# TheoCoombes/ClipCap

Hardware: AMD Instinct MI355X
Metric: train samples/sec (512-d prefix, 40-tok caption) (higher is better)
Workload: dtype bf16; 1 GPU; BASELINE configs[1]: TransformerMapper(8L,P=L=10,H=8)+frozen GPT-2-small; per_gpu_batch=256, global_batch=256, encoder_dim=512, train_language_model=False, parallelism=dp1

## Files before the change

clipcap_amd/csrc/kernels.hip:

```cpp
#include "kernels.h"
#include "gemm_api.h"

namespace CC_NS {

__global__ void k_f32_to_bf16(const float* __restrict__ src, op16_t* __restrict__ dst, size_t n8) {
    for (size_t i = (size_t)blockIdx.x * blockDim.x + threadIdx.x; i < n8; i += (size_t)gridDim.x * blockDim.x) {
        const float4 a = reinterpret_cast<const float4*>(src)[2 * i], b = reinterpret_cast<const float4*>(src)[2 * i + 1];
        float v[8] = {a.x, a.y, a.z, a.w, b.x, b.y, b.z, b.w};
        reinterpret_cast<uint4*>(dst)[i] = pack8(v);
    }
}
int f32_to_bf16(const float* src, op16_t* dst, size_t n, hipStream_t st) {
    if (n & 7) return CC_ERR_SHAPE;
    const size_t n8 = n >> 3;
    if (!n8) return CC_OK;
    const int grid = (int)std::min<size_t>((n8 + 255) / 256, 2048);
    hipLaunchKernelGGL(k_f32_to_bf16, dim3(grid), dim3(256), 0, st, src, dst, n8);
    return CC_OK;
}

__device__ __forceinline__ unsigned short wire_bf16(float f) {
    const unsigned u = __float_as_uint(f);
    if ((u & 0x7fffffffu) > 0x7f800000u) return (unsigned short)((u >> 16) | 0x40u);
    return (unsigned short)((u + 0x7fffu + ((u >> 16) & 1u)) >> 16);
// ... 1046 lines not shown
                    const op16x8 a_h = frag_row_p(Dh + (blk * 32 + l31) * LDP + j * 32, t, half), a_l = frag_row_p(Dl + (blk * 32 + l31) * LDP + j * 32, t, half);
                    const op16x8 b_h = frag_tr_p<LD>(Kh + j * 32 * LD, nb, t, lane), b_l = frag_tr_p<LD>(Kl + j * 32 * LD, nb, t, lane);
                    CC_MFMA3(a_h, a_l, b_h, b_l, acc)
                }
        } else {
            const op16_t* Ah = kind == 1 ? Dh : Ph, *Al = kind == 1 ? Dl : Pl, *Bh = kind == 1 ? Qh : Oh, *Bl = kind == 1 ? Ql : Ol;
            for (int i = CAUSAL ? blk : 0; i < NBLK; i++)
#pragma unroll
                for (int t = 0; t < 2; t++) {
                    const op16x8 a_h = frag_tr_p<LDP>(Ah + i * 32 * LDP, blk, t, lane), a_l = frag_tr_p<LDP>(Al + i * 32 * LDP, blk, t, lane);
                    const op16x8 b_h = frag_tr_p<LD>(Bh + i * 32 * LD, nb, t, lane), b_l = frag_tr_p<LD>(Bl + i * 32 * LD, nb, t, lane);
                    CC_MFMA3(a_h, a_l, b_h, b_l, acc)
                }
        }
        const int d = nb * 32 + l31;
        if (img) {
            const int odd = lane & 1;
            op16_t* r3 = reinterpret_cast<op16_t*>(dqkv) + (size_t)b * S * 9 * D + kind * D + h * HD + (d & ~1);
#pragma unroll
            for (int rp = 0; rp < 8; rp++) {
                const float v0 = acc[2 * rp], v1 = acc[2 * rp + 1];
                const float got = __shfl_xor(odd ? v0 : v1, 1, 64);
                const float a0 = odd ? got : v0, a1 = odd ? v1 : got;
                const int row = blk * 32 + ((2 * rp) & 3) + 8 * ((2 * rp) >> 2) + 4 * half + odd;
                const unsigned hi = pack2op(a0, a1);
                float h0, h1;
                unpack2(hi, h0, h1);
                const unsigned lo = pack2op(a0 - h0, a1 - h1);
                if (row < S) {
                    op16_t* o3 = r3 + (size_t)row * 9 * D;
                    *reinterpret_cast<unsigned*>(o3) = hi;
                    *reinterpret_cast<unsigned*>(o3 + 3 * D) = hi;
                    *reinterpret_cast<unsigned*>(o3 + 6 * D) = lo;
                }
            }
        } else {
            float* o1 = dqkv + (size_t)b * S * rs + kind * D + h * HD + d;
#pragma unroll
            for (int r = 0; r < 16; r++) {
                const int row = blk * 32 + (r & 3) + 8 * (r >> 2) + 4 * half;
                if (row < S) o1[(size_t)row * rs] = acc[r];
            }
        }
    }
    __syncthreads();
    }
}
template <int HD, int NBLK>
static int attn_bwd_m3_launch(const float* qkv, const float* dout, const float* lse, int B, int S, int H, bool causal, float* dqkv, hipStream_t st,
                              Drop drop, int img) {
    typedef AttM3<HD, NBLK> G;
    const float scale = 1.0f / sqrtf((float)HD);
    static int ncu = 0;
    if (!ncu) {
        int dev = 0;
        hipDeviceProp_t pr;
        if (hipGetDevice(&dev) != hipSuccess || hipGetDeviceProperties(&pr, dev) != hipSuccess) return CC_ERR_STATE;
        ncu = pr.multiProcessorCount;
    }
    const int per_cu = (int)((size_t)160 * 1024 / G::lds);
    const dim3 grid(min(B * H, ncu * max(1, per_cu))), blk(64 * G::NW);
#define CC_M3_LAUNCH(C, DR)                                                                                                              \
    {                                                                                                                                    \
        if (G::lds > 64 * 1024) (void)hipFuncSetAttribute((const void*)k_attn_bwd_m3<HD, NBLK, C, DR>, hipFuncAttributeMaxDynamicSharedMemorySize, (int)G::lds); \
        hipLaunchKernelGGL((k_attn_bwd_m3<HD, NBLK, C, DR>), grid, blk, G::lds, st, qkv, dout, lse, B, S, H, scale, dqkv, drop, img);          \
    }
    if (drop.thresh) {
        if (!causal) return CC_ERR_SHAPE;
        CC_M3_LAUNCH(true, true)
    } else if (causal) CC_M3_LAUNCH(true, false)
    else CC_M3_LAUNCH(false, false)
#undef CC_M3_LAUNCH
    return hipGetLastError() == hipSuccess ? CC_OK : CC_ERR_LAUNCH;
}
static bool attn_x3mfma_on();
static bool attn_bwd_m3_ok(int S, int hd) { return attn_x3mfma_on() && (hd == 64 || hd == 96) && S > 0 && S <= 64; }
static bool attn_x3mfma_on() {
    static const bool on = !(cc_lab_env("CC_ATTN_X3MFMA") && atoi(cc_lab_env("CC_ATTN_X3MFMA")) == 0) && !cc_lab_env("CC_ATTN_F32MFMA");
    return on;
}
#endif

#if CC_OP != 2
template <int HD, bool CAUSAL, bool DROP = false>
__global__ __launch_bounds__(256, HD == 64 ? 3 : 2) void k_attn_fwd_mfma(const op16_t* __restrict__ qkv, int B, int S, int H, float scale,
                                                       op16_t* __restrict__ out, float* __restrict__ lse_out, Drop drop = Drop()) {
    constexpr int KK = HD / 16, NB = HD / 32, C8 = HD / 8;
    __shared__ __attribute__((aligned(16))) op16_t vsm[4][32 * AttLd<HD>::v];
    const int lane = threadIdx.x & 63, wave = threadIdx.x >> 6;
    const int nqb = (S + 31) >> 5;
    const int item = blockIdx.x * 4 + wave;
    if (item >= B * H * nqb) return;
    const int qb = item % nqb, h = (item / nqb) % H, b = item / (nqb * H);
    const int D = H * HD;
    const size_t rs = (size_t)3 * D;
    const op16_t* base = qkv + (size_t)b * S * rs + h * HD;
    const int half = lane >> 5, q = qb * 32 + (lane & 31);
    op16_t* vs = vsm[wave];

    op16x8 qf[KK];
#pragma unroll
    for (int kk = 0; kk < KK; kk++) {
        uint4 v = *reinterpret_cast<const uint4*>(base + (size_t)min(q, S - 1) * rs + kk * 16 + half * 8);
        if (q >= S) v = make_uint4(0, 0, 0, 0);
        qf[kk] = __builtin_bit_cast(op16x8, v);
    }
    f32x16 o[NB];
#pragma unroll
    for (int nb = 0; nb < NB; nb++)
#pragma unroll
        for (int r = 0; r < 16; r++) o[nb][r] = 0.f;
    float m = -INFINITY, l = 0.f;
    const int nkb = CAUSAL ? qb + 1 : nqb;
    uint4 kq[KK], vq[HD / 16];
    auto fetch = [&](int kb, uint4 (&kd)[KK], uint4 (&vd)[HD / 16]) {
        const int key = kb * 32 + (lane & 31);
#pragma unroll
        for (int kk = 0; kk < KK; kk++) {
            kd[kk] = *reinterpret_cast<const uint4*>(base + D + (size_t)min(key, S - 1) * rs + kk * 16 + half * 8);
            if (key >= S) kd[kk] = make_uint4(0, 0, 0, 0);
        }
#pragma unroll
        for (int c = 0; c < HD / 16; c++) {
            const int idx = lane + 64 * c;
            const int vk = idx / C8, vc = idx % C8;
            vd[c] = *reinterpret_cast<const uint4*>(base + 2 * D + (size_t)min(kb * 32 + vk, S - 1) * rs + vc * 8);
            if (kb * 32 + vk >= S) vd[c] = make_uint4(0, 0, 0, 0);
        }
    };
    fetch(0, kq, vq);
    for (int kb = 0; kb < nkb; kb++) {
        uint4 kn[KK], vn[HD / 16];
        fetch(kb + 1, kn, vn);
        f32x16 s;
#pragma unroll
        for (int r = 0; r < 16; r++) s[r] = 0.f;
#pragma unroll
        for (int kk = 0; kk < KK; kk++) s = CC_MFMA_32x32x16(__builtin_bit_cast(op16x8, kq[kk]), qf[kk], s);
#pragma unroll
        for (int c = 0; c < HD / 16; c++) {
            const int idx = lane + 64 * c;
            *reinterpret_cast<uint4*>(vs + (idx / C8) * AttLd<HD>::v + (idx % C8) * 8) = vq[c];
        }
        float mx = -INFINITY;
#pragma unroll
        for (int r = 0; r < 16; r++) {
            const int kr = kb * 32 + (r & 3) + 8 * (r >> 2) + 4 * half;
            const bool ok = kr < S && (!CAUSAL || kr <= q);
            s[r] = ok ? s[r] * scale : -INFINITY;
            mx = fmaxf(mx, s[r]);
        }
        mx = fmaxf(mx, __shfl_xor(mx, 32, 64));
        const float m_new = fmaxf(m, mx);
        const float alpha = (m == -INFINITY) ? 0.f : __expf(m - m_new);
        float p[16], ps = 0.f;
#pragma unroll
        for (int r = 0; r < 16; r++) {
            p[r] = (m_new == -INFINITY) ? 0.f : __expf(s[r] - m_new);
            ps += p[r];
        }
        ps += __shfl_xor(ps, 32, 64);
        l = l * alpha + ps;
        m = m_new;
#pragma unroll
        for (int nb = 0; nb < NB; nb++)
#pragma unroll
            for (int r = 0; r < 16; r++) o[nb][r] *= alpha;
        if (DROP) {
            const unsigned rowbase = ((unsigned)(b * H + h) * S + min(q, S - 1)) * S;
#pragma unroll
            for (int r = 0; r < 16; r++) p[r] *= drop_mul(drop, rowbase + min(kb * 32 + (r & 3) + 8 * (r >> 2) + 4 * half, S - 1));
        }
        op16x8 pf[2];
#pragma unroll
        for (int t = 0; t < 2; t++) {
            const uint4 v = make_uint4(pack2op(p[t * 8 + 0], p[t * 8 + 1]), pack2op(p[t * 8 + 2], p[t * 8 + 3]),
                                       pack2op(p[t * 8 + 4], p[t * 8 + 5]), pack2op(p[t * 8 + 6], p[t * 8 + 7]));
            pf[t] = __builtin_bit_cast(op16x8, v);
        }
#pragma unroll
        for (int t = 0; t < 2; t++)
#pragma unroll
            for (int nb = 0; nb < NB; nb++) o[nb] = CC_MFMA_32x32x16(frag_tr<HD>(vs, nb, t, lane), pf[t], o[nb]);
#pragma unroll
        for (int kk = 0; kk < KK; kk++) kq[kk] = kn[kk];
#pragma unroll
        for (int c = 0; c < HD / 16; c++) vq[c] = vn[c];
    }
    if (q < S) {
        const float inv = l > 0.f ? 1.f / l : 0.f;
        op16_t* orow = out + ((size_t)b * S + q) * D + h * HD;
#pragma unroll
        for (int nb = 0; nb < NB; nb++)
#pragma unroll
            for (int g = 0; g < 4; g++) {
                const int d0 = nb * 32 + 8 * g + 4 * half;
                *reinterpret_cast<uint2*>(orow + d0) = make_uint2(pack2op(o[nb][g * 4 + 0] * inv, o[nb][g * 4 + 1] * inv),
                                                                  pack2op(o[nb][g * 4 + 2] * inv, o[nb][g * 4 + 3] * inv));
            }
        if (half == 0 && lse_out) lse_out[((size_t)b * H + h) * S + q] = m + __logf(l);
    }
}

template <int HD>
static int attn_fwd_mfma_launch(const op16_t* qkv, int B, int S, int H, bool causal, op16_t* out, float* lse, hipStream_t st, Drop drop) {
    const int items = B * H * ((S + 31) / 32);
    const float scale = 1.0f / sqrtf((float)HD);
    if (drop.thresh) {
        if (!causal) return CC_ERR_SHAPE;
        hipLaunchKernelGGL((k_attn_fwd_mfma<HD, true, true>), dim3((items + 3) / 4), dim3(256), 0, st, qkv, B, S, H, scale, out, lse, drop);
    } else if (causal)
        hipLaunchKernelGGL((k_attn_fwd_mfma<HD, true>), dim3((items + 3) / 4), dim3(256), 0, st, qkv, B, S, H, scale, out, lse, drop);
    else
        hipLaunchKernelGGL((k_attn_fwd_mfma<HD, false>), dim3((items + 3) / 4), dim3(256), 0, st, qkv, B, S, H, scale, out, lse, drop);
    return hipGetLastError() == hipSuccess ? CC_OK : CC_ERR_LAUNCH;
}

__device__ __forceinline__ op16x8 pack_frag(const float* p) {
    return __builtin_bit_cast(op16x8, make_uint4(pack2op(p[0], p[1]), pack2op(p[2], p[3]), pack2op(p[4], p[5]), pack2op(p[6], p[7])));
}
__device__ __forceinline__ op16x8 load_frag(const op16_t* row_ptr, bool ok) {
    uint4 v = *reinterpret_cast<const uint4*>(row_ptr);
    if (!ok) v = make_uint4(0, 0, 0, 0);
    return __builtin_bit_cast(op16x8, v);
}

template <int HD, bool CAUSAL, bool DROP = false>
__global__ __launch_bounds__(256, HD == 64 ? 2 : 1) void k_attn_bwd_dkv(const op16_t* __restrict__ qkv, const op16_t* __restrict__ dout,
                                                      const float* __restrict__ lse, const float* __restrict__ delta, int B, int S, int H,
                                                      float scale, op16_t* __restrict__ dqkv, Drop drop = Drop()) {
    constexpr int KK = HD / 16, NB = HD / 32;
    __shared__ __attribute__((aligned(16))) op16_t qsm[4][32 * AttLd<HD>::v];
    __shared__ __attribute__((aligned(16))) op16_t dsm[4][32 * AttLd<HD>::v];
    __shared__ __attribute__((aligned(16))) float ldsm[4][64];
    const int lane = threadIdx.x & 63, wave = threadIdx.x >> 6;
    const int nblk = (S + 31) >> 5;
    const int item = blockIdx.x * 4 + wave;
    if (item >= B * H * nblk) return;
    const int j = item % nblk, h = (item / nblk) % H, b = item / (nblk * H);
    const int D = H * HD;
    const size_t rs = (size_t)3 * D;
    const op16_t* base = qkv + (size_t)b * S * rs + h * HD;
    const op16_t* dbase = dout + (size_t)b * S * D + h * HD;
    const float* lrow = lse + ((size_t)b * H + h) * S;
    const float* drow = delta + ((size_t)b * H + h) * S;
    const int half = lane >> 5, key = j * 32 + (lane & 31);
    op16x8 kf[KK], vf[KK];
#pragma unroll
    for (int kk = 0; kk < KK; kk++) {
        kf[kk] = load_frag(base + D + (size_t)min(key, S - 1) * rs + kk * 16 + half * 8, key < S);
        vf[kk] = load_frag(base + 2 * D + (size_t)min(key, S - 1) * rs + kk * 16 + half * 8, key < S);
    }
    f32x16 dk[NB], dv[NB];
#pragma unroll
    for (int nb = 0; nb < NB; nb++)
#pragma unroll
        for (int r = 0; r < 16; r++) { dk[nb][r] = 0.f; dv[nb][r] = 0.f; }
    const int i0 = CAUSAL ? j : 0;
    op16x8 qf[KK], df[KK];
    {
        const int qa = i0 * 32 + (lane & 31);
#pragma unroll
        for (int kk = 0; kk < KK; kk++) {
            qf[kk] = load_frag(base + (size_t)min(qa, S - 1) * rs + kk * 16 + half * 8, qa < S);
            df[kk] = load_frag(dbase + (size_t)min(qa, S - 1) * D + kk * 16 + half * 8, qa < S);
        }
    }
    for (int i = i0; i < nblk; i++) {
        op16x8 qn[KK], dn[KK];
        {
            const int qa = (i + 1) * 32 + (lane & 31);
#pragma unroll
            for (int kk = 0; kk < KK; kk++) {
                qn[kk] = load_frag(base + (size_t)min(qa, S - 1) * rs + kk * 16 + half * 8, qa < S);
                dn[kk] = load_frag(dbase + (size_t)min(qa, S - 1) * D + kk * 16 + half * 8, qa < S);
            }
        }
        f32x16 s, dp;
#pragma unroll
        for (int r = 0; r < 16; r++) { s[r] = 0.f; dp[r] = 0.f; }
#pragma unroll
        for (int kk = 0; kk < KK; kk++) {
            s = CC_MFMA_32x32x16(qf[kk], kf[kk], s);
            dp = CC_MFMA_32x32x16(df[kk], vf[kk], dp);
            *reinterpret_cast<op16x8*>(qsm[wave] + (lane & 31) * AttLd<HD>::v + kk * 16 + half * 8) = qf[kk];
            *reinterpret_cast<op16x8*>(dsm[wave] + (lane & 31) * AttLd<HD>::v + kk * 16 + half * 8) = df[kk];
        }
        {
            const int qq = min(i * 32 + (lane & 31), S - 1);
            ldsm[wave][lane] = half ? drow[qq] : lrow[qq];
        }
        float lq[16], dq_[16];
// ... 81 lines not shown
#pragma unroll
    for (int nb = 0; nb < NB; nb++)
#pragma unroll
        for (int r = 0; r < 16; r++) dq[nb][r] = 0.f;
    const int jend = CAUSAL ? i + 1 : nblk;
    op16x8 kf[KK], vf[KK];
    {
        const int key = lane & 31;
#pragma unroll
        for (int kk = 0; kk < KK; kk++) {
            kf[kk] = load_frag(base + D + (size_t)min(key, S - 1) * rs + kk * 16 + half * 8, key < S);
            vf[kk] = load_frag(base + 2 * D + (size_t)min(key, S - 1) * rs + kk * 16 + half * 8, key < S);
        }
    }
    for (int j = 0; j < jend; j++) {
        op16x8 kn[KK], vn[KK];
        {
            const int key = (j + 1) * 32 + (lane & 31);
#pragma unroll
            for (int kk = 0; kk < KK; kk++) {
                kn[kk] = load_frag(base + D + (size_t)min(key, S - 1) * rs + kk * 16 + half * 8, key < S);
                vn[kk] = load_frag(base + 2 * D + (size_t)min(key, S - 1) * rs + kk * 16 + half * 8, key < S);
            }
        }
        f32x16 st, dpt;
#pragma unroll
        for (int r = 0; r < 16; r++) { st[r] = 0.f; dpt[r] = 0.f; }
#pragma unroll
        for (int kk = 0; kk < KK; kk++) {
            st = CC_MFMA_32x32x16(kf[kk], qf[kk], st);
            dpt = CC_MFMA_32x32x16(vf[kk], dof[kk], dpt);
            *reinterpret_cast<op16x8*>(ksm[wave] + (lane & 31) * AttLd<HD>::v + kk * 16 + half * 8) = kf[kk];
        }
        float ds[16];
#pragma unroll
        for (int r = 0; r < 16; r++) {
            const int kr = j * 32 + (r & 3) + 8 * (r >> 2) + 4 * half;
            const bool ok = kr < S && q < S && (!CAUSAL || kr <= q);
            const float p = ok ? __expf(st[r] * scale - my_lse) : 0.f;
            const float mk = DROP ? drop_mul(drop, ((unsigned)(b * H + h) * S + min(q, S - 1)) * S + min(kr, S - 1)) : 1.0f;
            ds[r] = p * (mk * dpt[r] - my_delta) * scale;
        }
        const op16x8 dsf[2] = {pack_frag(ds), pack_frag(ds + 8)};
#pragma unroll
        for (int t = 0; t < 2; t++)
#pragma unroll
            for (int nb = 0; nb < NB; nb++)
                dq[nb] = CC_MFMA_32x32x16(frag_tr<HD>(ksm[wave], nb, t, lane), dsf[t], dq[nb]);
#pragma unroll
        for (int kk = 0; kk < KK; kk++) { kf[kk] = kn[kk]; vf[kk] = vn[kk]; }
    }
    if (q < S) {
        op16_t* orow = dqkv + ((size_t)b * S + q) * rs + h * HD;
#pragma unroll
        for (int nb = 0; nb < NB; nb++)
#pragma unroll
            for (int g = 0; g < 4; g++) {
                const int d0 = nb * 32 + 8 * g + 4 * half;
                *reinterpret_cast<uint2*>(orow + d0) =
                    make_uint2(pack2op(dq[nb][g * 4 + 0], dq[nb][g * 4 + 1]), pack2op(dq[nb][g * 4 + 2], dq[nb][g * 4 + 3]));
            }
    }
}

#ifndef CC_ATTN_FUSED_OCC
#define CC_ATTN_FUSED_OCC 2
#endif
template <int LD, int ROWS = 32>
__device__ __forceinline__ op16x8 frag_tr_ld(const op16_t* blk, int nb, int t, int lane) {
    typedef __attribute__((ext_vector_type(4))) short s16x4_t;
    typedef __attribute__((address_space(3))) s16x4_t* lp_t;
    const int half = lane >> 5, j = lane & 15, dsub = (lane >> 4) & 1;
    const int r0 = 16 * t + 4 * half + (j >> 2);
    const op16_t* col = blk + nb * 32 + 16 * dsub + 4 * (j & 3);
    const op16_t* p = col + (ROWS < 32 ? min(r0, ROWS - 1) : r0) * LD;
    const op16_t* ph = col + (ROWS < 32 ? min(r0 + 8, ROWS - 1) : r0 + 8) * LD;
    const s16x4_t lo = __builtin_amdgcn_ds_read_tr16_b64_v4i16((lp_t)p);
    const s16x4_t hi = __builtin_amdgcn_ds_read_tr16_b64_v4i16((lp_t)ph);
    typedef __attribute__((ext_vector_type(8))) short s16x8_t;
    const s16x8_t v = {lo[0], lo[1], lo[2], lo[3], hi[0], hi[1], hi[2], hi[3]};
    return __builtin_bit_cast(op16x8, v);
}

template <int HD>
__device__ __forceinline__ void attn_store_tile(op16_t* T, const f32x16 (&acc)[HD / 32], op16_t* gblock, size_t gstride, int rows_left, int lane) {
    constexpr int LD = AttLd<HD>::v, C8 = HD / 8;
    const int half = lane >> 5, l31 = lane & 31;
#pragma unroll
    for (int nb = 0; nb < HD / 32; nb++)
#pragma unroll
        for (int g = 0; g < 4; g++)
            *reinterpret_cast<uint2*>(T + l31 * LD + nb * 32 + 8 * g + 4 * half) =
                make_uint2(pack2op(acc[nb][g * 4 + 0], acc[nb][g * 4 + 1]), pack2op(acc[nb][g * 4 + 2], acc[nb][g * 4 + 3]));
#pragma unroll
    for (int it = 0; it < C8 / 2; it++) {
        const int idx = lane + 64 * it, row = idx / C8, chunk = idx % C8;
        const uint4 v = *reinterpret_cast<const uint4*>(T + row * LD + chunk * 8);
        if (row < rows_left) *reinterpret_cast<uint4*>(gblock + (size_t)row * gstride + chunk * 8) = v;
    }
}

template <int HD, bool CAUSAL, bool DROP, int NBLK, int OCC, int DR = 32>
__global__ __launch_bounds__(256, OCC) void k_attn_bwd_fused(const op16_t* __restrict__ qkv, const op16_t* __restrict__ dout, const op16_t* __restrict__ o,
                                                             const float* __restrict__ lse, int B, int S, int H, float scale,
                                                             op16_t* __restrict__ dqkv, Drop drop = Drop()) {
    constexpr int KK = HD / 16, NB = HD / 32, LD = AttLd<HD>::v;
    constexpr bool SPARE = LD >= HD + 32;
    constexpr int LT = SPARE ? LD : 32;
    __shared__ __attribute__((aligned(16))) op16_t ksm[4][32 * LD];
    __shared__ __attribute__((aligned(16))) op16_t qsm[4][32 * LD];
    __shared__ __attribute__((aligned(16))) op16_t dsm[4][32 * LD];
    static_assert(DR == 32 || (!SPARE && NBLK == 1), "the short dS^T tile is for the single-block form with its own tile");
    __shared__ __attribute__((aligned(16))) op16_t dtx[SPARE ? 1 : 4][SPARE ? 8 : DR * 32];
    __shared__ __attribute__((aligned(16))) float ldsm[4][NBLK][64];
    const int lane = threadIdx.x & 63, wave = threadIdx.x >> 6;
    const int item = blockIdx.x * 4 + wave;
    if (item >= B * H) return;
    const int h = item % H, b = item / H;
    const int D = H * HD;
    const size_t rs = (size_t)3 * D;
    const op16_t* base = qkv + (size_t)b * S * rs + h * HD;
    const op16_t* dbase = dout + (size_t)b * S * D + h * HD;
    const op16_t* obase = o + (size_t)b * S * D + h * HD;
    const float* lrow = lse + ((size_t)b * H + h) * S;
    const int half = lane >> 5, l31 = lane & 31;
    const int coff = half * 8;
    op16_t* dtm = SPARE ? ksm[wave] + HD : dtx[SPARE ? 0 : wave];

    op16x8 qf[KK], dof[KK], kf[KK], vf[KK];
    auto load_q = [&](int i) {
        const int q = i * 32 + l31, qc = min(q, S - 1);
#pragma unroll
        for (int kk = 0; kk < KK; kk++) {
            qf[kk] = load_frag(base + (size_t)qc * rs + kk * 16 + coff, q < S);
            dof[kk] = load_frag(dbase + (size_t)qc * D + kk * 16 + coff, q < S);
        }
    };
    auto load_k = [&](int j) {
        const int key = j * 32 + l31, kc = min(key, S - 1);
#pragma unroll
        for (int kk = 0; kk < KK; kk++) {
            kf[kk] = load_frag(base + D + (size_t)kc * rs + kk * 16 + coff, key < S);
            vf[kk] = load_frag(base + 2 * D + (size_t)kc * rs + kk * 16 + coff, key < S);
        }
    };
    load_k(0);
    load_q(0);
#pragma unroll
    for (int i = 0; i < NBLK; i++) {
        const int q = i * 32 + l31, qc = min(q, S - 1);
        float acc = 0.f;
#pragma unroll
        for (int kk = 0; kk < KK; kk++) {
            const op16x8 df = load_frag(dbase + (size_t)qc * D + kk * 16 + coff, q < S);
            const op16x8 of = load_frag(obase + (size_t)qc * D + kk * 16 + coff, q < S);
            float x[8], y[8];
            unpack8(__builtin_bit_cast(uint4, df), x);
            unpack8(__builtin_bit_cast(uint4, of), y);
#pragma unroll
            for (int e = 0; e < 8; e++) acc += x[e] * y[e];
        }
        acc += __shfl_xor(acc, 32, 64);
        ldsm[wave][i][lane] = half ? acc : lrow[qc];
    }
    f32x16 dq[NBLK][NB];

#pragma unroll
    for (int j = 0; j < NBLK; j++) {
        const int key = j * 32 + l31;
#pragma unroll
        for (int kk = 0; kk < KK; kk++) *reinterpret_cast<op16x8*>(ksm[wave] + l31 * LD + kk * 16 + coff) = kf[kk];
        f32x16 dk[NB], dv[NB];
#pragma unroll
        for (int nb = 0; nb < NB; nb++)
#pragma unroll
            for (int r = 0; r < 16; r++) { dk[nb][r] = 0.f; dv[nb][r] = 0.f; }
#pragma unroll
        for (int i = 0; i < NBLK; i++) {
            if (CAUSAL && i < j) continue;
            const int ifirst = CAUSAL ? j : 0;
            if (!(j > 0 && i == ifirst && i == NBLK - 1)) {
#pragma unroll
                for (int kk = 0; kk < KK; kk++) {
                    *reinterpret_cast<op16x8*>(qsm[wave] + l31 * LD + kk * 16 + coff) = qf[kk];
                    *reinterpret_cast<op16x8*>(dsm[wave] + l31 * LD + kk * 16 + coff) = dof[kk];
                }
            }
            f32x16 s, dp;
#pragma unroll
            for (int r = 0; r < 16; r++) { s[r] = 0.f; dp[r] = 0.f; }
#pragma unroll
            for (int kk = 0; kk < KK; kk++) {
                s = CC_MFMA_32x32x16(qf[kk], kf[kk], s);
                dp = CC_MFMA_32x32x16(dof[kk], vf[kk], dp);
            }
            if (i + 1 < NBLK) {
                load_q(i + 1);
            } else if (j + 1 < NBLK) {
                const int ni = CAUSAL ? j + 1 : 0;
                if (ni != i) load_q(ni);
                load_k(j + 1);
            }
            if (j == 0) {
#pragma unroll
                for (int nb = 0; nb < NB; nb++)
#pragma unroll
                    for (int r = 0; r < 16; r++) dq[i][nb][r] = 0.f;
            }
            float p[16], ds[16];
#pragma unroll
            for (int g4 = 0; g4 < 4; g4++) {
                const float4 lq = *reinterpret_cast<const float4*>(&ldsm[wave][i][4 * half + 8 * g4]);
                const float4 dl = *reinterpret_cast<const float4*>(&ldsm[wave][i][32 + 4 * half + 8 * g4]);
                const float lqa[4] = {lq.x, lq.y, lq.z, lq.w}, dla[4] = {dl.x, dl.y, dl.z, dl.w};
#pragma unroll
                for (int e = 0; e < 4; e++) {
                    const int r = g4 * 4 + e;
                    const int qr = i * 32 + e + 8 * g4 + 4 * half;
                    const bool ok = qr < S && key < S && (!CAUSAL || key <= qr);
                    p[r] = ok ? __expf(s[r] * scale - lqa[e]) : 0.f;
                    if (DROP) {
                        const float mk = drop_mul(drop, ((unsigned)(b * H + h) * S + min(qr, S - 1)) * S + min(key, S - 1));
                        ds[r] = p[r] * (mk * dp[r] - dla[e]) * scale;
                        p[r] *= mk;
                    } else {
                        ds[r] = p[r] * (dp[r] - dla[e]) * scale;
                    }
                }
            }
            const op16x8 pf[2] = {pack_frag(p), pack_frag(p + 8)};
            const op16x8 dsf[2] = {pack_frag(ds), pack_frag(ds + 8)};
            if (DR == 32 || l31 < DR) {
#pragma unroll
                for (int t = 0; t < 2; t++) {
                    const uint4 w = __builtin_bit_cast(uint4, dsf[t]);
                    *reinterpret_cast<uint2*>(dtm + l31 * LT + 16 * t + 4 * half) = make_uint2(w.x, w.y);
                    *reinterpret_cast<uint2*>(dtm + l31 * LT + 16 * t + 8 + 4 * half) = make_uint2(w.z, w.w);
                }
            }
#pragma unroll
            for (int t = 0; t < 2; t++)
#pragma unroll
                for (int nb = 0; nb < NB; nb++) {
                    dv[nb] = CC_MFMA_32x32x16(frag_tr<HD>(dsm[wave], nb, t, lane), pf[t], dv[nb]);
                    dk[nb] = CC_MFMA_32x32x16(frag_tr<HD>(qsm[wave], nb, t, lane), dsf[t], dk[nb]);
                }
#pragma unroll
            for (int t = 0; t < 2; t++) {
                const op16x8 dst = frag_tr_ld<LT, DR>(dtm, 0, t, lane);
#pragma unroll
                for (int nb = 0; nb < NB; nb++) dq[i][nb] = CC_MFMA_32x32x16(frag_tr<HD>(ksm[wave], nb, t, lane), dst, dq[i][nb]);
            }
            if (j == (CAUSAL ? i : NBLK - 1)) {
                attn_store_tile<HD>(qsm[wave], dq[i], dqkv + ((size_t)b * S + i * 32) * rs + h * HD, rs, S - i * 32, lane);
            }
        }
        {
            op16_t* gblk = dqkv + ((size_t)b * S + j * 32) * rs + h * HD;
            attn_store_tile<HD>(ksm[wave], dk, gblk + D, rs, S - j * 32, lane);
            attn_store_tile<HD>(ksm[wave], dv, gblk + 2 * D, rs, S - j * 32, lane);
        }
    }
}

template <int HD, int NBLK>
static void attn_bwd_fused_launch(const op16_t* qkv, const op16_t* dout, const op16_t* o, const float* lse, int B, int S, int H, bool causal,
                                  op16_t* dqkv, hipStream_t st, Drop drop, float scale) {
    constexpr int OCC = CC_ATTN_FUSED_OCC;
    const dim3 grid((B * H + 3) / 4), blk(256);
    if (drop.thresh) hipLaunchKernelGGL((k_attn_bwd_fused<HD, true, true, NBLK, (HD == 64 ? OCC : 1)>), grid, blk, 0, st, qkv, dout, o, lse, B, S, H, scale, dqkv, drop);
    else if (causal) hipLaunchKernelGGL((k_attn_bwd_fused<HD, true, false, NBLK, (HD == 64 ? OCC : 1)>), grid, blk, 0, st, qkv, dout, o, lse, B, S, H, scale, dqkv, drop);
    else {
        if constexpr (HD == 96 && NBLK == 1) {
            static const bool short_on = []() { const char* e = cc_lab_env("CC_ATTN_BWD_SHORT"); return !e || atoi(e) != 0; }();
            if (S <= 24 && short_on) {
                hipLaunchKernelGGL((k_attn_bwd_fused<HD, false, false, NBLK, 2, 24>), grid, blk, 0, st, qkv, dout, o, lse, B, S, H, scale, dqkv, drop);
                return;
            }
        }
        hipLaunchKernelGGL((k_attn_bwd_fused<HD, false, false, NBLK, 1>), grid, blk, 0, st, qkv, dout, o, lse, B, S, H, scale, dqkv, drop);
    }
}

template <int HD>
static int attn_bwd_mfma_launch(const op16_t* qkv, const op16_t* dout, const op16_t* o, const float* lse, float* delta, int B, int S, int H,
                                bool causal, op16_t* dqkv, hipStream_t st, Drop drop) {
    const int items = B * H * ((S + 31) / 32);
    const float scale = 1.0f / sqrtf((float)HD);
    if (drop.thresh && !causal) return CC_ERR_SHAPE;
    static const int fused = []() { const char* e = cc_lab_env("CC_ATTN_BWD_FUSED"); return e ? atoi(e) : 1; }();
    if (fused && S <= 32) {
        attn_bwd_fused_launch<HD, 1>(qkv, dout, o, lse, B, S, H, causal, dqkv, st, drop, scale);
        return hipGetLastError() == hipSuccess ? CC_OK : CC_ERR_LAUNCH;
    }
    if constexpr (HD < 128) {
        if (fused && S <= 64) {
            attn_bwd_fused_launch<HD, 2>(qkv, dout, o, lse, B, S, H, causal, dqkv, st, drop, scale);
            return hipGetLastError() == hipSuccess ? CC_OK : CC_ERR_LAUNCH;
        }
    }
    if (drop.thresh) {
        hipLaunchKernelGGL((k_attn_bwd_dq<HD, true, true>), dim3((items + 3) / 4), dim3(256), 0, st, qkv, dout, o, lse, delta, B, S, H, scale, dqkv, drop);
        hipLaunchKernelGGL((k_attn_bwd_dkv<HD, true, true>), dim3((items + 3) / 4), dim3(256), 0, st, qkv, dout, lse, delta, B, S, H, scale, dqkv, drop);
    } else if (causal) {
        hipLaunchKernelGGL((k_attn_bwd_dq<HD, true>), dim3((items + 3) / 4), dim3(256), 0, st, qkv, dout, o, lse, delta, B, S, H, scale, dqkv);
        hipLaunchKernelGGL((k_attn_bwd_dkv<HD, true>), dim3((items + 3) / 4), dim3(256), 0, st, qkv, dout, lse, delta, B, S, H, scale, dqkv);
    } else {
        hipLaunchKernelGGL((k_attn_bwd_dq<HD, false>), dim3((items + 3) / 4), dim3(256), 0, st, qkv, dout, o, lse, delta, B, S, H, scale, dqkv);
        hipLaunchKernelGGL((k_attn_bwd_dkv<HD, false>), dim3((items + 3) / 4), dim3(256), 0, st, qkv, dout, lse, delta, B, S, H, scale, dqkv);
    }
    return hipGetLastError() == hipSuccess ? CC_OK : CC_ERR_LAUNCH;
}

#endif

static size_t attn_fwd_lds(int S, int hd) { return ((size_t)3 * S * (hd + 4) + (size_t)S * (S + 1)) * 4; }
static size_t attn_bwd_lds(int S, int hd) {
    if (S < 32) return ((size_t)4 * S * (hd + 4) + (size_t)2 * S * (S + 1)) * 4;
    const size_t S4 = (S + 3) & ~3;
    return ((size_t)4 * S4 * (hd + 4) + (size_t)2 * S4 * (S4 + 4)) * 4;
}

__global__ __launch_bounds__(256) void k_attn_probs(const act_t* __restrict__ qkv, int B, int S, int H, int hd, float scale,
                                                    float* __restrict__ out) {
    const int wave = blockIdx.x * 4 + (threadIdx.x >> 6), lane = threadIdx.x & 63;
    if (wave >= B * H * S) return;
    const int n = wave % S, h = (wave / S) % H, b = wave / (S * H);
    const int D = H * hd;
    const act_t* q = qkv + ((size_t)b * S + n) * 3 * D + h * hd;
    float mx = -INFINITY;
    for (int m0 = 0; m0 < S; m0 += 64) {
        const int m = m0 + lane;
        float sc = -INFINITY;
        if (m < S) {
            const act_t* k = qkv + ((size_t)b * S + m) * 3 * D + D + h * hd;
            float acc = 0.f;
            for (int d = 0; d < hd; d++) acc += act2f(q[d]) * act2f(k[d]);
            sc = acc * scale;
            out[(((size_t)b * S + n) * S + m) * H + h] = sc;
        }
        mx = fmaxf(mx, wave_max(sc));
    }
    float sum = 0.f;
    for (int m = lane; m < S; m += 64) sum += __expf(out[(((size_t)b * S + n) * S + m) * H + h] - mx);
    sum = wave_sum(sum);
    for (int m = lane; m < S; m += 64) {
        float* o = out + (((size_t)b * S + n) * S + m) * H + h;
        *o = __expf(*o - mx) / sum;
    }
}
int attn_probs(const act_t* qkv, int B, int S, int H, int hd, float* out, hipStream_t st) {
    const int waves = B * H * S;
    if (waves <= 0) return CC_OK;
    hipLaunchKernelGGL(k_attn_probs, dim3((waves + 3) / 4), dim3(256), 0, st, qkv, B, S, H, hd, 1.0f / sqrtf((float)hd), out);
    return CC_OK;
}

#if CC_OP == 2
__device__ __forceinline__ float row_dot(const float* a, const float* b, int hd) {
    float s0 = 0.f, s1 = 0.f;
    for (int d = 0; d < hd; d += 8) {
        const float4 x0 = *reinterpret_cast<const float4*>(a + d), y0 = *reinterpret_cast<const float4*>(b + d);
        const float4 x1 = *reinterpret_cast<const float4*>(a + d + 4), y1 = *reinterpret_cast<const float4*>(b + d + 4);
        s0 += x0.x * y0.x + x0.y * y0.y + x0.z * y0.z + x0.w * y0.w;
        s1 += x1.x * y1.x + x1.y * y1.y + x1.z * y1.z + x1.w * y1.w;
    }
    return s0 + s1;
}
template <bool CAUSAL>
__global__ __launch_bounds__(256) void k_attn_fwd_rows(const float* __restrict__ qkv, int B, int S, int H, int hd, float scale, float* __restrict__ out,
                                                       float* __restrict__ lse) {
    extern __shared__ float rsm[];
    const int lane = threadIdx.x & 63, wave = threadIdx.x >> 6;
    const int item = blockIdx.x * 4 + wave;
    if (item >= B * H * S) return;
    const int i = item % S, h = (item / S) % H, b = item / (S * H);
    const int D = H * hd;
    const size_t rs = (size_t)3 * D;
    const float* base = qkv + (size_t)b * S * rs + h * hd;
    const float* q = base + (size_t)i * rs;
    float* p = rsm + wave * S;
// ... 1489 lines not shown
```

Before: 22460 samples/s.

## Load attention Q/K/V tiles as coalesced rows and restage fragments through LDS

The MFMA attention forward kernel now loads Q, K and V as whole contiguous row chunks spread across lanes instead of per-lane fragment-strided reads. It stages them through shared memory to build MFMA fragments, and writes the output tile back through LDS with full-row stores. The same row-load path is added to the fused backward kernel but only behind an experiment flag. The goal is better global-memory coalescing in exchange for extra LDS traffic, an extra per-wave LDS buffer that may affect occupancy, and restructured prefetching.

After: 22590 samples/s, median of 6. No clear change (+0.6%).

```diff
diff --git a/clipcap_amd/csrc/kernels.hip b/clipcap_amd/csrc/kernels.hip
--- a/clipcap_amd/csrc/kernels.hip
+++ b/clipcap_amd/csrc/kernels.hip
@@ -1152,11 +1152,62 @@
 #endif
 
 #if CC_OP != 2
-template <int HD, bool CAUSAL, bool DROP = false>
+template <int HD>
+__device__ __forceinline__ void attn_load_rows(const op16_t* gcol, size_t gstride, int row0, int S, int lane, uint4 (&d)[HD / 16]) {
+    constexpr int C8 = HD / 8;
+#pragma unroll
+    for (int c = 0; c < HD / 16; c++) {
+        const int idx = lane + 64 * c, row = row0 + idx / C8;
+        d[c] = *reinterpret_cast<const uint4*>(gcol + (size_t)min(row, S - 1) * gstride + (idx % C8) * 8);
+        if (row >= S) d[c] = make_uint4(0, 0, 0, 0);
+    }
+}
+template <int HD>
+__device__ __forceinline__ void attn_put_rows(op16_t* T, const uint4 (&d)[HD / 16], int lane) {
+    constexpr int C8 = HD / 8;
+#pragma unroll
+    for (int c = 0; c < HD / 16; c++) {
+        const int idx = lane + 64 * c;
+        *reinterpret_cast<uint4*>(T + (idx / C8) * AttLd<HD>::v + (idx % C8) * 8) = d[c];
+    }
+}
+template <int HD>
+__device__ __forceinline__ void attn_get_frags(const op16_t* T, int lane, op16x8 (&f)[HD / 16]) {
+#pragma unroll
+    for (int kk = 0; kk < HD / 16; kk++) f[kk] = *reinterpret_cast<const op16x8*>(T + (lane & 31) * AttLd<HD>::v + kk * 16 + (lane >> 5) * 8);
+}
+
+template <int HD>
+__device__ __forceinline__ void attn_store_tile(op16_t* T, const f32x16 (&acc)[HD / 32], op16_t* gblock, size_t gstride, int rows_left, int lane) {
+    constexpr int LD = AttLd<HD>::v, C8 = HD / 8;
+    const int half = lane >> 5, l31 = lane & 31;
+#pragma unroll
+    for (int nb = 0; nb < HD / 32; nb++)
+#pragma unroll
+        for (int g = 0; g < 4; g++)
+            *reinterpret_cast<uint2*>(T + l31 * LD + nb * 32 + 8 * g + 4 * half) =
+                make_uint2(pack2op(acc[nb][g * 4 + 0], acc[nb][g * 4 + 1]), pack2op(acc[nb][g * 4 + 2], acc[nb][g * 4 + 3]));
+#pragma unroll
+    for (int it = 0; it < C8 / 2; it++) {
+        const int idx = lane + 64 * it, row = idx / C8, chunk = idx % C8;
+        const uint4 v = *reinterpret_cast<const uint4*>(T + row * LD + chunk * 8);
+        if (row < rows_left) *reinterpret_cast<uint4*>(gblock + (size_t)row * gstride + chunk * 8) = v;
+    }
+}
+
+#ifdef CC_EXPERIMENTS
+static int attn_lines() {
+    static const int v = []() { const char* e = cc_lab_env("CC_ATTN_LINES"); return e ? atoi(e) : 1; }();
+    return v;
+}
+#endif
+
+template <int HD, bool CAUSAL, bool DROP = false, bool LINES = true>
 __global__ __launch_bounds__(256, HD == 64 ? 3 : 2) void k_attn_fwd_mfma(const op16_t* __restrict__ qkv, int B, int S, int H, float scale,
                                                        op16_t* __restrict__ out, float* __restrict__ lse_out, Drop drop = Drop()) {
     constexpr int KK = HD / 16, NB = HD / 32, C8 = HD / 8;
     __shared__ __attribute__((aligned(16))) op16_t vsm[4][32 * AttLd<HD>::v];
+    __shared__ __attribute__((aligned(16))) op16_t ksm[LINES ? 4 : 1][LINES ? 32 * AttLd<HD>::v : 8];
     const int lane = threadIdx.x & 63, wave = threadIdx.x >> 6;
     const int nqb = (S + 31) >> 5;
     const int item = blockIdx.x * 4 + wave;
@@ -1169,11 +1220,16 @@
     op16_t* vs = vsm[wave];
 
     op16x8 qf[KK];
-#pragma unroll
-    for (int kk = 0; kk < KK; kk++) {
-        uint4 v = *reinterpret_cast<const uint4*>(base + (size_t)min(q, S - 1) * rs + kk * 16 + half * 8);
-        if (q >= S) v = make_uint4(0, 0, 0, 0);
-        qf[kk] = __builtin_bit_cast(op16x8, v);
+    uint4 qst[KK];
+    if constexpr (LINES) {
+        attn_load_rows<HD>(base, rs, qb * 32, S, lane, qst);
+    } else {
+#pragma unroll
+        for (int kk = 0; kk < KK; kk++) {
+            uint4 v = *reinterpret_cast<const uint4*>(base + (size_t)min(q, S - 1) * rs + kk * 16 + half * 8);
+            if (q >= S) v = make_uint4(0, 0, 0, 0);
+            qf[kk] = __builtin_bit_cast(op16x8, v);
+        }
     }
     f32x16 o[NB];
 #pragma unroll
@@ -1184,6 +1240,11 @@
     const int nkb = CAUSAL ? qb + 1 : nqb;
     uint4 kq[KK], vq[HD / 16];
     auto fetch = [&](int kb, uint4 (&kd)[KK], uint4 (&vd)[HD / 16]) {
+        if constexpr (LINES) {
+            attn_load_rows<HD>(base + D, rs, kb * 32, S, lane, kd);
+            attn_load_rows<HD>(base + 2 * D, rs, kb * 32, S, lane, vd);
+            return;
+        }
         const int key = kb * 32 + (lane & 31);
 #pragma unroll
         for (int kk = 0; kk < KK; kk++) {
@@ -1199,18 +1260,34 @@
         }
     };
     fetch(0, kq, vq);
+    if constexpr (LINES) {
+        attn_put_rows<HD>(vs, qst, lane);
+        attn_get_frags<HD>(vs, lane, qf);
+    }
     for (int kb = 0; kb < nkb; kb++) {
         uint4 kn[KK], vn[HD / 16];
-        fetch(kb + 1, kn, vn);
+        op16x8 kf[KK];
+        if constexpr (LINES) {
+            attn_put_rows<HD>(ksm[wave], kq, lane);
+            attn_put_rows<HD>(vs, vq, lane);
+            if (kb + 1 < nkb) fetch(kb + 1, kq, vq);
+            attn_get_frags<HD>(ksm[wave], lane, kf);
+        } else {
+            fetch(kb + 1, kn, vn);
+#pragma unroll
+            for (int kk = 0; kk < KK; kk++) kf[kk] = __builtin_bit_cast(op16x8, kq[kk]);
+        }
         f32x16 s;
 #pragma unroll
         for (int r = 0; r < 16; r++) s[r] = 0.f;
 #pragma unroll
-        for (int kk = 0; kk < KK; kk++) s = CC_MFMA_32x32x16(__builtin_bit_cast(op16x8, kq[kk]), qf[kk], s);
-#pragma unroll
-        for (int c = 0; c < HD / 16; c++) {
-            const int idx = lane + 64 * c;
-            *reinterpret_cast<uint4*>(vs + (idx / C8) * AttLd<HD>::v + (idx % C8) * 8) = vq[c];
+        for (int kk = 0; kk < KK; kk++) s = CC_MFMA_32x32x16(kf[kk], qf[kk], s);
+        if constexpr (!LINES) {
+#pragma unroll
+            for (int c = 0; c < HD / 16; c++) {
+                const int idx = lane + 64 * c;
+                *reinterpret_cast<uint4*>(vs + (idx / C8) * AttLd<HD>::v + (idx % C8) * 8) = vq[c];
+            }
         }
         float mx = -INFINITY;
 #pragma unroll
@@ -1252,22 +1329,33 @@
         for (int t = 0; t < 2; t++)
 #pragma unroll
             for (int nb = 0; nb < NB; nb++) o[nb] = CC_MFMA_32x32x16(frag_tr<HD>(vs, nb, t, lane), pf[t], o[nb]);
-#pragma unroll
-        for (int kk = 0; kk < KK; kk++) kq[kk] = kn[kk];
-#pragma unroll
-        for (int c = 0; c < HD / 16; c++) vq[c] = vn[c];
+        if constexpr (!LINES) {
+#pragma unroll
+            for (int kk = 0; kk < KK; kk++) kq[kk] = kn[kk];
+#pragma unroll
+            for (int c = 0; c < HD / 16; c++) vq[c] = vn[c];
+        }
+    }
+    const float inv = l > 0.f ? 1.f / l : 0.f;
+    if constexpr (LINES) {
+#pragma unroll
+        for (int nb = 0; nb < NB; nb++)
+#pragma unroll
+            for (int r = 0; r < 16; r++) o[nb][r] *= inv;
+        attn_store_tile<HD>(vs, o, out + ((size_t)b * S + qb * 32) * D + h * HD, D, S - qb * 32, lane);
     }
     if (q < S) {
-        const float inv = l > 0.f ? 1.f / l : 0.f;
-        op16_t* orow = out + ((size_t)b * S + q) * D + h * HD;
-#pragma unroll
-        for (int nb = 0; nb < NB; nb++)
-#pragma unroll
-            for (int g = 0; g < 4; g++) {
-                const int d0 = nb * 32 + 8 * g + 4 * half;
-                *reinterpret_cast<uint2*>(orow + d0) = make_uint2(pack2op(o[nb][g * 4 + 0] * inv, o[nb][g * 4 + 1] * inv),
-                                                                  pack2op(o[nb][g * 4 + 2] * inv, o[nb][g * 4 + 3] * inv));
-            }
+        if constexpr (!LINES) {
+            op16_t* orow = out + ((size_t)b * S + q) * D + h * HD;
+#pragma unroll
+            for (int nb = 0; nb < NB; nb++)
+#pragma unroll
+                for (int g = 0; g < 4; g++) {
+                    const int d0 = nb * 32 + 8 * g + 4 * half;
+                    *reinterpret_cast<uint2*>(orow + d0) = make_uint2(pack2op(o[nb][g * 4 + 0] * inv, o[nb][g * 4 + 1] * inv),
+                                                                      pack2op(o[nb][g * 4 + 2] * inv, o[nb][g * 4 + 3] * inv));
+                }
+        }
         if (half == 0 && lse_out) lse_out[((size_t)b * H + h) * S + q] = m + __logf(l);
     }
 }
@@ -1276,8 +1364,19 @@
 static int attn_fwd_mfma_launch(const op16_t* qkv, int B, int S, int H, bool causal, op16_t* out, float* lse, hipStream_t st, Drop drop) {
     const int items = B * H * ((S + 31) / 32);
     const float scale = 1.0f / sqrtf((float)HD);
+    if (drop.thresh && !causal) return CC_ERR_SHAPE;
+#ifdef CC_EXPERIMENTS
+    if (!attn_lines()) {
+        if (drop.thresh)
+            hipLaunchKernelGGL((k_attn_fwd_mfma<HD, true, true, false>), dim3((items + 3) / 4), dim3(256), 0, st, qkv, B, S, H, scale, out, lse, drop);
+        else if (causal)
+            hipLaunchKernelGGL((k_attn_fwd_mfma<HD, true, false, false>), dim3((items + 3) / 4), dim3(256), 0, st, qkv, B, S, H, scale, out, lse, drop);
+        else
+            hipLaunchKernelGGL((k_attn_fwd_mfma<HD, false, false, false>), dim3((items + 3) / 4), dim3(256), 0, st, qkv, B, S, H, scale, out, lse, drop);
+        return hipGetLastError() == hipSuccess ? CC_OK : CC_ERR_LAUNCH;
+    }
+#endif
     if (drop.thresh) {
-        if (!causal) return CC_ERR_SHAPE;
         hipLaunchKernelGGL((k_attn_fwd_mfma<HD, true, true>), dim3((items + 3) / 4), dim3(256), 0, st, qkv, B, S, H, scale, out, lse, drop);
     } else if (causal)
         hipLaunchKernelGGL((k_attn_fwd_mfma<HD, true>), dim3((items + 3) / 4), dim3(256), 0, st, qkv, B, S, H, scale, out, lse, drop);
@@ -1525,25 +1624,7 @@
     return __builtin_bit_cast(op16x8, v);
 }
 
-template <int HD>
-__device__ __forceinline__ void attn_store_tile(op16_t* T, const f32x16 (&acc)[HD / 32], op16_t* gblock, size_t gstride, int rows_left, int lane) {
-    constexpr int LD = AttLd<HD>::v, C8 = HD / 8;
-    const int half = lane >> 5, l31 = lane & 31;
-#pragma unroll
-    for (int nb = 0; nb < HD / 32; nb++)
-#pragma unroll
-        for (int g = 0; g < 4; g++)
-            *reinterpret_cast<uint2*>(T + l31 * LD + nb * 32 + 8 * g + 4 * half) =
-                make_uint2(pack2op(acc[nb][g * 4 + 0], acc[nb][g * 4 + 1]), pack2op(acc[nb][g * 4 + 2], acc[nb][g * 4 + 3]));
-#pragma unroll
-    for (int it = 0; it < C8 / 2; it++) {
-        const int idx = lane + 64 * it, row = idx / C8, chunk = idx % C8;
-        const uint4 v = *reinterpret_cast<const uint4*>(T + row * LD + chunk * 8);
-        if (row < rows_left) *reinterpret_cast<uint4*>(gblock + (size_t)row * gstride + chunk * 8) = v;
-    }
-}
-
-template <int HD, bool CAUSAL, bool DROP, int NBLK, int OCC, int DR = 32>
+template <int HD, bool CAUSAL, bool DROP, int NBLK, int OCC, int DR = 32, bool LINES = false>
 __global__ __launch_bounds__(256, OCC) void k_attn_bwd_fused(const op16_t* __restrict__ qkv, const op16_t* __restrict__ dout, const op16_t* __restrict__ o,
                                                              const float* __restrict__ lse, int B, int S, int H, float scale,
                                                              op16_t* __restrict__ dqkv, Drop drop = Drop()) {
@@ -1587,32 +1668,61 @@
             vf[kk] = load_frag(base + 2 * D + (size_t)kc * rs + kk * 16 + coff, key < S);
         }
     };
-    load_k(0);
-    load_q(0);
-#pragma unroll
-    for (int i = 0; i < NBLK; i++) {
-        const int q = i * 32 + l31, qc = min(q, S - 1);
+    uint4 kst[KK], vst[KK], qst[KK], dst[KK], ost[KK];
+    auto fetch_q = [&](int i, bool with_o) {
+        attn_load_rows<HD>(base, rs, i * 32, S, lane, qst);
+        attn_load_rows<HD>(dbase, D, i * 32, S, lane, dst);
+        if (with_o) attn_load_rows<HD>(obase, D, i * 32, S, lane, ost);
+    };
+    auto fetch_k = [&](int j) {
+        attn_load_rows<HD>(base + D, rs, j * 32, S, lane, kst);
+        attn_load_rows<HD>(base + 2 * D, rs, j * 32, S, lane, vst);
+    };
+    auto put_delta = [&](int i, const op16x8 (&df)[KK], const op16x8 (&of)[KK]) {
         float acc = 0.f;
 #pragma unroll
         for (int kk = 0; kk < KK; kk++) {
-            const op16x8 df = load_frag(dbase + (size_t)qc * D + kk * 16 + coff, q < S);
-            const op16x8 of = load_frag(obase + (size_t)qc * D + kk * 16 + coff, q < S);
             float x[8], y[8];
-            unpack8(__builtin_bit_cast(uint4, df), x);
-            unpack8(__builtin_bit_cast(uint4, of), y);
+            unpack8(__builtin_bit_cast(uint4, df[kk]), x);
+            unpack8(__builtin_bit_cast(uint4, of[kk]), y);
 #pragma unroll
             for (int e = 0; e < 8; e++) acc += x[e] * y[e];
         }
         acc += __shfl_xor(acc, 32, 64);
-        ldsm[wave][i][lane] = half ? acc : lrow[qc];
+        ldsm[wave][i][lane] = half ? acc : lrow[min(i * 32 + l31, S - 1)];
+    };
+    if constexpr (LINES) {
+        fetch_k(0);
+        fetch_q(0, true);
+    } else {
+        load_k(0);
+        load_q(0);
+#pragma unroll
+        for (int i = 0; i < NBLK; i++) {
+            const int q = i * 32 + l31, qc = min(q, S - 1);
+            op16x8 df[KK], of[KK];
+#pragma unroll
+            for (int kk = 0; kk < KK; kk++) {
+                df[kk] = load_frag(dbase + (size_t)qc * D + kk * 16 + coff, q < S);
+                of[kk] = load_frag(obase + (size_t)qc * D + kk * 16 + coff, q < S);
+            }
+            put_delta(i, df, of);
+        }
     }
     f32x16 dq[NBLK][NB];
 
 #pragma unroll
     for (int j = 0; j < NBLK; j++) {
         const int key = j * 32 + l31;
-#pragma unroll
-        for (int kk = 0; kk < KK; kk++) *reinterpret_cast<op16x8*>(ksm[wave] + l31 * LD + kk * 16 + coff) = kf[kk];
+        if constexpr (LINES) {
+            attn_put_rows<HD>(ksm[wave], vst, lane);
+            attn_get_frags<HD>(ksm[wave], lane, vf);
+            attn_put_rows<HD>(ksm[wave], kst, lane);
+            attn_get_frags<HD>(ksm[wave], lane, kf);
+        } else {
+#pragma unroll
+            for (int kk = 0; kk < KK; kk++) *reinterpret_cast<op16x8*>(ksm[wave] + l31 * LD + kk * 16 + coff) = kf[kk];
+        }
         f32x16 dk[NB], dv[NB];
 #pragma unroll
         for (int nb = 0; nb < NB; nb++)
@@ -1623,10 +1733,23 @@
             if (CAUSAL && i < j) continue;
             const int ifirst = CAUSAL ? j : 0;
             if (!(j > 0 && i == ifirst && i == NBLK - 1)) {
-#pragma unroll
-                for (int kk = 0; kk < KK; kk++) {
-                    *reinterpret_cast<op16x8*>(qsm[wave] + l31 * LD + kk * 16 + coff) = qf[kk];
-                    *reinterpret_cast<op16x8*>(dsm[wave] + l31 * LD + kk * 16 + coff) = dof[kk];
+                if constexpr (LINES) {
+                    op16x8 of[KK];
+                    if (j == 0) {
+                        attn_put_rows<HD>(qsm[wave], ost, lane);
+                        attn_get_frags<HD>(qsm[wave], lane, of);
+                    }
+                    attn_put_rows<HD>(qsm[wave], qst, lane);
+                    attn_put_rows<HD>(dsm[wave], dst, lane);
+                    attn_get_frags<HD>(qsm[wave], lane, qf);
+                    attn_get_frags<HD>(dsm[wave], lane, dof);
+                    if (j == 0) put_delta(i, dof, of);
+                } else {
+#pragma unroll
+                    for (int kk = 0; kk < KK; kk++) {
+                        *reinterpret_cast<op16x8*>(qsm[wave] + l31 * LD + kk * 16 + coff) = qf[kk];
+                        *reinterpret_cast<op16x8*>(dsm[wave] + l31 * LD + kk * 16 + coff) = dof[kk];
+                    }
                 }
             }
             f32x16 s, dp;
@@ -1638,11 +1761,16 @@
                 dp = CC_MFMA_32x32x16(dof[kk], vf[kk], dp);
             }
             if (i + 1 < NBLK) {
-                load_q(i + 1);
+                if constexpr (LINES) fetch_q(i + 1, j == 0); else load_q(i + 1);
             } else if (j + 1 < NBLK) {
                 const int ni = CAUSAL ? j + 1 : 0;
-                if (ni != i) load_q(ni);
-                load_k(j + 1);
+                if constexpr (LINES) {
+                    if (ni != i) fetch_q(ni, false);
+                    fetch_k(j + 1);
+                } else {
+                    if (ni != i) load_q(ni);
+                    load_k(j + 1);
+                }
             }
             if (j == 0) {
 #pragma unroll
@@ -1706,22 +1834,22 @@
     }
 }
 
-template <int HD, int NBLK>
+template <int HD, int NBLK, bool LINES = false>
 static void attn_bwd_fused_launch(const op16_t* qkv, const op16_t* dout, const op16_t* o, const float* lse, int B, int S, int H, bool causal,
                                   op16_t* dqkv, hipStream_t st, Drop drop, float scale) {
     constexpr int OCC = CC_ATTN_FUSED_OCC;
     const dim3 grid((B * H + 3) / 4), blk(256);
-    if (drop.thresh) hipLaunchKernelGGL((k_attn_bwd_fused<HD, true, true, NBLK, (HD == 64 ? OCC : 1)>), grid, blk, 0, st, qkv, dout, o, lse, B, S, H, scale, dqkv, drop);
-    else if (causal) hipLaunchKernelGGL((k_attn_bwd_fused<HD, true, false, NBLK, (HD == 64 ? OCC : 1)>), grid, blk, 0, st, qkv, dout, o, lse, B, S, H, scale, dqkv, drop);
+    if (drop.thresh) hipLaunchKernelGGL((k_attn_bwd_fused<HD, true, true, NBLK, (HD == 64 ? OCC : 1), 32, LINES>), grid, blk, 0, st, qkv, dout, o, lse, B, S, H, scale, dqkv, drop);
+    else if (causal) hipLaunchKernelGGL((k_attn_bwd_fused<HD, true, false, NBLK, (HD == 64 ? OCC : 1), 32, LINES>), grid, blk, 0, st, qkv, dout, o, lse, B, S, H, scale, dqkv, drop);
     else {
         if constexpr (HD == 96 && NBLK == 1) {
             static const bool short_on = []() { const char* e = cc_lab_env("CC_ATTN_BWD_SHORT"); return !e || atoi(e) != 0; }();
             if (S <= 24 && short_on) {
-                hipLaunchKernelGGL((k_attn_bwd_fused<HD, false, false, NBLK, 2, 24>), grid, blk, 0, st, qkv, dout, o, lse, B, S, H, scale, dqkv, drop);
+                hipLaunchKernelGGL((k_attn_bwd_fused<HD, false, false, NBLK, 2, 24, LINES>), grid, blk, 0, st, qkv, dout, o, lse, B, S, H, scale, dqkv, drop);
                 return;
             }
         }
-        hipLaunchKernelGGL((k_attn_bwd_fused<HD, false, false, NBLK, 1>), grid, blk, 0, st, qkv, dout, o, lse, B, S, H, scale, dqkv, drop);
+        hipLaunchKernelGGL((k_attn_bwd_fused<HD, false, false, NBLK, 1, 32, LINES>), grid, blk, 0, st, qkv, dout, o, lse, B, S, H, scale, dqkv, drop);
     }
 }
 
@@ -1732,14 +1860,30 @@
     const float scale = 1.0f / sqrtf((float)HD);
     if (drop.thresh && !causal) return CC_ERR_SHAPE;
     static const int fused = []() { const char* e = cc_lab_env("CC_ATTN_BWD_FUSED"); return e ? atoi(e) : 1; }();
-    if (fused && S <= 32) {
-        attn_bwd_fused_launch<HD, 1>(qkv, dout, o, lse, B, S, H, causal, dqkv, st, drop, scale);
-        return hipGetLastError() == hipSuccess ? CC_OK : CC_ERR_LAUNCH;
-    }
-    if constexpr (HD < 128) {
-        if (fused && S <= 64) {
-            attn_bwd_fused_launch<HD, 2>(qkv, dout, o, lse, B, S, H, causal, dqkv, st, drop, scale);
+#ifdef CC_EXPERIMENTS
+    if (attn_lines() >= 2) {
+        if (fused && S <= 32) {
+            attn_bwd_fused_launch<HD, 1, true>(qkv, dout, o, lse, B, S, H, causal, dqkv, st, drop, scale);
             return hipGetLastError() == hipSuccess ? CC_OK : CC_ERR_LAUNCH;
+        }
+        if constexpr (HD < 128) {
+            if (fused && S <= 64) {
+                attn_bwd_fused_launch<HD, 2, true>(qkv, dout, o, lse, B, S, H, causal, dqkv, st, drop, scale);
+                return hipGetLastError() == hipSuccess ? CC_OK : CC_ERR_LAUNCH;
+            }
+        }
+    } else
+#endif
+    {
+        if (fused && S <= 32) {
+            attn_bwd_fused_launch<HD, 1>(qkv, dout, o, lse, B, S, H, causal, dqkv, st, drop, scale);
+            return hipGetLastError() == hipSuccess ? CC_OK : CC_ERR_LAUNCH;
+        }
+        if constexpr (HD < 128) {
+            if (fused && S <= 64) {
+                attn_bwd_fused_launch<HD, 2>(qkv, dout, o, lse, B, S, H, causal, dqkv, st, drop, scale);
+                return hipGetLastError() == hipSuccess ? CC_OK : CC_ERR_LAUNCH;
+            }
         }
     }
     if (drop.thresh) {
```
